# cr1m5onk1ng/text_similarity

Hardware: AMD Instinct MI355X
Metric: sentences/sec encoded + Mpairs/sec cosine top-k @ N=1M d=384 (higher is better)
Workload: dtype bf16 encoder / f16 selection / fp32 scores

## Files before the change

### include/tsim.h

```cpp
#ifndef TSIM_H
#define TSIM_H

#include <stddef.h>
#include <stdint.h>

#ifdef __cplusplus
extern "C" {
#endif

#define TSIM_OK 0
#define TSIM_EINVAL 1
#define TSIM_EHIP 2
#define TSIM_ENOMEM 3
#define TSIM_EUNSUPPORTED 4

#define TSIM_F32 0
#define TSIM_BF16 1

#define TSIM_ARCH_BERT 0
#define TSIM_ARCH_MPNET 1
#define TSIM_ARCH_ROBERTA 2

int tsim_version(void);
const char *tsim_last_error(void);
// ... 213 lines not shown
#define TSIM_POOL_MEAN_SQRT_LEN 3
#define TSIM_ACT_IDENTITY 0
#define TSIM_ACT_TANH 1
#define TSIM_ACT_RELU 2
typedef struct tsim_sentence_head {
    int32_t pool_mode;
    int32_t d_out;
    const float *dense_w, *dense_b;
    int32_t dense_act;
    int32_t normalize;
} tsim_sentence_head;

int tsim_encoder_forward_head(tsim_encoder *enc, const int32_t *tok_ids, const int32_t *tok_type, const int32_t *tok_pos,
                              const int32_t *tok_col, const int32_t *cu_seqlens, int32_t T, int32_t B, int32_t max_len,
                              const tsim_sentence_head *head, float *emb_f32, void *unit_f16, int ld_unit,
                              float *unit_rho_max, void *last_hidden_bf16, void *stream);

int tsim_encoder_forward_spans(tsim_encoder *enc, const int32_t *tok_ids, const int32_t *tok_type, const int32_t *tok_pos,
                               const int32_t *tok_col, const int32_t *cu_seqlens, int32_t T, int32_t B, int32_t max_len,
                               float *pooled_f32, void *unit_f16, int ld_unit, float *unit_rho_max,
                               void *last_hidden_bf16, float *logits_f32, const int32_t *span_seq, const int32_t *span_cu,
                               const int32_t *span_tok, int32_t S, int32_t n_span_tok, float *span_out_f32,
                               void *span_unit_f16, int ld_span_unit, float *span_rho_max, void *stream);

#define TSIM_ENC_ERR_TOKEN_ID 1
#define TSIM_ENC_ERR_POSITION 2
#define TSIM_ENC_ERR_MAX_LEN 4
#define TSIM_ENC_ERR_TOKEN_TYPE 8
#define TSIM_ENC_ERR_SPAN 16
int tsim_encoder_error_flags(tsim_encoder *enc, int32_t *flags_host, void *stream);

int tsim_chain_items_host(int blocks, int rem_blocks, int ntiles, int G, int b, int32_t *items, int cap);

int tsim_wordpiece_create(const char *vocab_text, const int64_t *vocab_offsets, int32_t vocab_size,
                          const char *continuing_prefix, int32_t unk_id, const int32_t *prefix_ids, int32_t n_prefix,
                          const int32_t *suffix_ids, int32_t n_suffix, int32_t lowercase, int32_t max_input_chars_per_word,
                          const char *added_text, const int64_t *added_offsets, int32_t n_added, void **handle);
void tsim_wordpiece_destroy(void *handle);
int tsim_wordpiece_encode(void *handle, const char *text, const int64_t *text_offsets, int64_t n, int32_t max_len,
                          int32_t n_threads, int32_t *out_ids, int64_t out_capacity, int32_t *out_lens, uint8_t *handled);

#ifdef __cplusplus
}
#endif
#endif
```

### text_similarity_amd/_lib.py

```python
from __future__ import annotations

import ctypes as C
import os

_HERE = os.path.dirname(os.path.abspath(__file__))
LIB_PATH = os.environ.get("TSIM_LIB") or os.path.join(_HERE, "libtsim.so")

TSIM_F32, TSIM_BF16 = 0, 1
TSIM_I32, TSIM_I64 = 2, 3
LIST_ST_ROW, LIST_ST_LIMS = 1, 2
IVF_ST_LIST, IVF_ST_OFF = 1, 2
IVF_SEG = 512
ARCH_BERT, ARCH_MPNET, ARCH_ROBERTA = 0, 1, 2
W_BF16, W_MXFP8 = 0, 1
POOL_MEAN, POOL_CLS, POOL_MAX, POOL_MEAN_SQRT_LEN = 0, 1, 2, 3
ACT_IDENTITY, ACT_TANH, ACT_RELU = 0, 1, 2
SPACE_COSINE, SPACE_DOT, SPACE_L2 = 0, 1, 2
ENC_ERR_SPAN = 16
RANGE_SLOT_CAP = 2048
RANGE_MERGE_MAX_LISTS = 64


class TsimError(RuntimeError):
    pass
# ... 108 lines not shown
                                    C.c_void_p, C.c_int64, C.c_void_p, C.c_size_t, C.c_void_p]),
    "tsim_int8_rescore_topk": (C.c_int, [C.c_void_p, C.c_int64, C.c_int64, C.c_void_p, C.c_int64, C.c_int64, C.c_int, C.c_void_p,
                                         C.c_int64, C.c_int, C.c_void_p, C.c_void_p, C.c_int64, C.c_void_p, C.c_void_p]),
    "tsim_ivf_scan_workspace_bytes": (C.c_size_t, [C.c_int64, C.c_int, C.c_int64, C.c_int]),
    "tsim_ivf_scan_topk": (C.c_int, [C.c_int, C.c_void_p, C.c_int64, C.c_int64, C.c_void_p, C.c_int64, C.c_int64, C.c_int, C.c_void_p,
                                     C.c_int64, C.c_void_p, C.c_void_p, C.c_int, C.c_int64, C.c_int, C.c_void_p, C.c_void_p, C.c_int64,
                                     C.c_void_p, C.c_void_p, C.c_size_t, C.c_void_p]),
    "tsim_cosine_topk": (C.c_int, [C.c_void_p, C.c_int64, C.c_void_p, C.c_int64, C.c_int, C.c_int, C.c_int,
                                   C.c_void_p, C.c_void_p, C.c_int64, C.c_void_p, C.c_size_t, C.c_void_p]),
    "tsim_time_next_topk": (None, [C.c_void_p, C.c_void_p]),
    "tsim_topk_merge": (C.c_int, [C.c_void_p, C.c_void_p, C.c_int, C.c_int64, C.c_int, C.c_int, C.c_void_p,
                                  C.c_void_p, C.c_void_p]),
    "tsim_topk_merge_strided": (C.c_int, [C.c_void_p, C.c_void_p, C.c_int, C.c_int64, C.c_int, C.c_int, C.c_int64, C.c_int64,
                                          C.c_void_p, C.c_void_p, C.c_void_p]),
    "tsim_wordpiece_create": (C.c_int, [C.c_char_p, C.c_void_p, C.c_int32, C.c_char_p, C.c_int32, C.c_void_p, C.c_int32, C.c_void_p,
                                        C.c_int32, C.c_int32, C.c_int32, C.c_char_p, C.c_void_p, C.c_int32, C.POINTER(C.c_void_p)]),
    "tsim_wordpiece_destroy": (None, [C.c_void_p]),
    "tsim_wordpiece_encode": (C.c_int, [C.c_void_p, C.c_char_p, C.c_void_p, C.c_int64, C.c_int32, C.c_int32, C.c_void_p, C.c_int64,
                                        C.c_void_p, C.c_void_p]),
    "tsim_cos_sim": (C.c_int, [C.c_void_p, C.c_int64, C.c_void_p, C.c_int64, C.c_int, C.c_void_p, C.c_void_p]),
    "tsim_mean_pool": (C.c_int, [C.c_void_p, C.c_int, C.c_void_p, C.c_int64, C.c_int, C.c_int, C.c_void_p,
                                 C.c_void_p]),
    "tsim_pool": (C.c_int, [C.c_void_p, C.c_int, C.c_void_p, C.c_int64, C.c_int, C.c_int, C.c_int, C.c_void_p, C.c_void_p]),
    "tsim_dense_rows": (C.c_int, [C.c_void_p, C.c_int64, C.c_int, C.c_void_p, C.c_void_p, C.c_int, C.c_int, C.c_int, C.c_void_p,
                                  C.c_void_p]),
    "tsim_quantize_mxfp8": (C.c_int, [C.c_void_p, C.c_int64, C.c_int, C.c_void_p, C.c_void_p, C.c_void_p]),
    "tsim_gemm_mxfp8": (C.c_int, [C.c_void_p, C.c_void_p, C.c_void_p, C.c_void_p, C.c_void_p, C.c_void_p, C.c_int, C.c_int,
                                  C.c_int, C.c_void_p]),
    "tsim_encoder_create": (C.c_int, [C.POINTER(EncoderConfigC), C.POINTER(EncoderWeightsC),
                                      C.POINTER(C.c_void_p)]),
    "tsim_encoder_destroy": (None, [C.c_void_p]),
    "tsim_encoder_error_flags": (C.c_int, [C.c_void_p, C.POINTER(C.c_int32), C.c_void_p]),
    "tsim_chain_items_host": (C.c_int, [C.c_int, C.c_int, C.c_int, C.c_int, C.c_int, C.POINTER(C.c_int32), C.c_int]),
    "tsim_encoder_forward": (C.c_int, [C.c_void_p, C.c_void_p, C.c_void_p, C.c_void_p, C.c_void_p, C.c_int32,
                                       C.c_int32, C.c_int32, C.c_void_p, C.c_void_p, C.c_int, C.c_void_p, C.c_void_p,
                                       C.c_void_p]),
    "tsim_encoder_set_token_types": (C.c_int, [C.c_void_p, C.c_void_p, C.c_int32]),
    "tsim_encoder_set_cls_head": (C.c_int, [C.c_void_p, C.c_void_p, C.c_void_p, C.c_void_p, C.c_void_p, C.c_int32]),
    "tsim_encoder_set_cls_head_act": (C.c_int, [C.c_void_p, C.c_void_p, C.c_void_p, C.c_void_p, C.c_void_p, C.c_int32, C.c_int32]),
    "tsim_encoder_forward_ex": (C.c_int, [C.c_void_p, C.c_void_p, C.c_void_p, C.c_void_p, C.c_void_p, C.c_void_p, C.c_int32,
                                          C.c_int32, C.c_int32, C.c_void_p, C.c_void_p, C.c_int, C.c_void_p, C.c_void_p,
                                          C.c_void_p, C.c_void_p]),
    "tsim_encoder_forward_head": (C.c_int, [C.c_void_p, C.c_void_p, C.c_void_p, C.c_void_p, C.c_void_p, C.c_void_p, C.c_int32,
                                            C.c_int32, C.c_int32, C.POINTER(SentenceHeadC), C.c_void_p, C.c_void_p, C.c_int,
                                            C.c_void_p, C.c_void_p, C.c_void_p]),
    "tsim_encoder_forward_spans": (C.c_int, [C.c_void_p, C.c_void_p, C.c_void_p, C.c_void_p, C.c_void_p, C.c_void_p, C.c_int32,
                                             C.c_int32, C.c_int32, C.c_void_p, C.c_void_p, C.c_int, C.c_void_p, C.c_void_p,
                                             C.c_void_p, C.c_void_p, C.c_void_p, C.c_void_p, C.c_int32, C.c_int32, C.c_void_p,
                                             C.c_void_p, C.c_int, C.c_void_p, C.c_void_p]),
}

DECLARED_SYMBOLS = tuple(_SIGS)


def lib() -> C.CDLL:
    global _lib
    if _lib is None:
        if not os.path.exists(LIB_PATH):
            raise TsimError(f"{LIB_PATH} not found: build it with `python -m text_similarity_amd.build` "
                            "(hipcc --offload-arch=gfx950); there is no CPU fallback")
        L = C.CDLL(LIB_PATH)
        for name, (res, args) in _SIGS.items():
            try:
                fn = getattr(L, name)
            except AttributeError:
                def fn(*a, _n=name, **kw):
# ... 15 lines not shown
```

### text_similarity_amd/csrc/encoder.hip

```cpp
#include <math.h>
#include <cmath>

#include <stdlib.h>
#include <string.h>

#include <vector>

#include <type_traits>
#include <utility>

#include "common.h"
#include "gemm_pp.h"

namespace tsim {

__device__ __forceinline__ int64_t packed_off(int64_t t, int f, int W) {
    return ((t >> 5) * (W >> 3) + (f >> 3)) * 256 + (t & 31) * 8 + (f & 7);
}
__device__ __forceinline__ int64_t group_off(int64_t t, int g, int W, int packed) {
    return packed ? packed_off(t, 8 * g, W) * 2 : (t * W + 8 * g) * 2;
}

template <int VPL, bool TYPED = false>
__global__ __launch_bounds__(256) void embed_ln_kernel(const int32_t *__restrict__ ids,
                                                       const int32_t *__restrict__ pos,
                                                       const float *__restrict__ word,
                                                       const float *__restrict__ pos_emb,
                                                       const float *__restrict__ type_tab,
                                                       const float *__restrict__ gamma,
                                                       const float *__restrict__ beta, float eps, int T, int H,
                                                       bf16_t *__restrict__ out, int vocab, int max_pos,
                                                       const int32_t *__restrict__ col, int max_len,
                                                       int *__restrict__ err_flags,
                                                       const int32_t *__restrict__ tok_type = nullptr, int n_types = 0) {
    const int lane = threadIdx.x & 63;
    const int t = blockIdx.x * 4 + (threadIdx.x >> 6);
    if (t >= T) return;
    int id = ids[t], ps = pos[t];
    int ty = 0;
    if constexpr (TYPED) ty = tok_type[t];
    int bad = 0;
    if (id < 0 || id >= vocab) { bad |= TSIM_ENC_ERR_TOKEN_ID; id = id < 0 ? 0 : vocab - 1; }
    if (ps < 0 || ps >= max_pos) { bad |= TSIM_ENC_ERR_POSITION; ps = ps < 0 ? 0 : max_pos - 1; }
    if (col[t] >= max_len || col[t] < 0) bad |= TSIM_ENC_ERR_MAX_LEN;
    if constexpr (TYPED) {
        if (ty < 0 || ty >= n_types) { bad |= TSIM_ENC_ERR_TOKEN_TYPE; ty = ty < 0 ? 0 : n_types - 1; }
    }
    if (bad && lane == 0) atomicOr(err_flags, bad);
    const float *w = word + (int64_t)id * H;
    const float *p = pos_emb + (int64_t)ps * H;
    const float *type_row = TYPED ? type_tab + (int64_t)ty * H : type_tab;
    float v[VPL], pv[VPL], tv[VPL];
#pragma unroll
    for (int i = 0; i < VPL; ++i) {
        v[i] = w[lane + i * 64];
        pv[i] = p[lane + i * 64];
    }
    if (type_row) {
#pragma unroll
        for (int i = 0; i < VPL; ++i) tv[i] = type_row[lane + i * 64];
    }
    float s = 0.f;
#pragma unroll
    for (int i = 0; i < VPL; ++i) {
        float a = v[i];
        if (type_row) a += tv[i];
        a += pv[i];
        v[i] = a;
        s += a;
// ... 1057 lines not shown
            }
            ++st;
            ring = ring + 1 == X2_NSTAGE ? 0 : ring + 1;
            if (st >= 3) carry = 0;
        }
        old_m0 = m0;
        old_n0 = n0;
        old_rowoff = (uint32_t)(m0 >> 5) * (uint32_t)(N2 * 64) + 16u * r2 + 512u * h2;
    };
    int item = 0;
    run_item(accA, accB, item++, std::false_type{});
    for (; item + 2 <= part.n; item += 2) {
        run_item(accB, accA, item, std::true_type{});
        run_item(accA, accB, item + 1, std::true_type{});
    }
    const bool lastA = item >= part.n;
    if (!lastA) run_item(accB, accA, item, std::true_type{});
    wait_vmcnt<0>();
    auto flush = [&](f32x16 (&a)[X2_NSUB]) __attribute__((always_inline)) {
#pragma unroll
        for (int g = 0; g < X2_NSUB; ++g) {
            uint32_t pk[8];
#pragma unroll
            for (int ks = 0; ks < 8; ++ks) pk[ks] = finish2(a[g][2 * ks], a[g][2 * ks + 1]);
            store_half(pk, old_m0, old_n0 + g * 32, std::integral_constant<int, 0>{});
            store_half(pk, old_m0, old_n0 + g * 32, std::integral_constant<int, 2>{});
        }
    };
    if (lastA) flush(accA); else flush(accB);
}

template <int DH, bool REL, bool PK = false>
__global__ __launch_bounds__(256) __attribute__((amdgpu_waves_per_eu(DH <= 32 ? 6 : 4))) void attention_kernel(const bf16_t *__restrict__ qkv,
                                                        const int32_t *__restrict__ cu, const int32_t *__restrict__ col,
                                                        const float *__restrict__ relb, int relw, int H,
                                                        int heads, float scale, bf16_t *__restrict__ ctx, int B, int xcd_map) {
    constexpr int KS = DH / 16;
    constexpr int OT = (DH + 31) / 32;
    constexpr int ROWB = DH * 2 < 64 ? 64 : DH * 2;
    __shared__ __attribute__((aligned(16))) char vimg[4 * 32 * ROWB];
    typedef __attribute__((ext_vector_type(4))) short s16x4;
    const int lane = threadIdx.x & 63;
    const int wave = __builtin_amdgcn_readfirstlane(threadIdx.x >> 6);
    int seq = blockIdx.x;
    if (xcd_map) {
        seq = (blockIdx.x & 7) * (gridDim.x >> 3) + (blockIdx.x >> 3);
        if (seq >= B) return;
    }
    const int head = blockIdx.y * 4 + wave, qb = blockIdx.z;
    const int t0 = cu[seq], S = cu[seq + 1] - t0;
    if (qb * 32 >= S || head >= heads) return;
    const int r = lane & 31, h = lane >> 5;
    const int64_t H3 = 3 * (int64_t)H;
    const int qi = qb * 32 + r;
    const int tq = t0 + (qi < S ? qi : S - 1);

    bf16x8 qf[KS];
    {
        const bf16_t *qp = PK ? qkv + packed_off(tq, head * DH + 8 * h, (int)H3) : qkv + tq * H3 + head * DH + 8 * h;
#pragma unroll
        for (int s = 0; s < KS; ++s) {
            qf[s] = *reinterpret_cast<const bf16x8 *>(qp + (PK ? 2 * 256 : 16) * s);
        }
    }
    const int qcol = REL ? col[tq] : 0;
    f32x16 o[OT];
#pragma unroll
    for (int ob = 0; ob < OT; ++ob)
#pragma unroll
        for (int g = 0; g < 16; ++g) o[ob][g] = 0.f;
    float m = -INFINITY, l = 0.f;

    for (int k0 = 0; k0 < S; k0 += 32) {
        const int kr = k0 + r;
        const int tk = t0 + (kr < S ? kr : S - 1);
        f32x16 sc;
#pragma unroll
        for (int g = 0; g < 16; ++g) sc[g] = 0.f;
        constexpr int CH = DH / 16;
        uint4 vr[CH];
        {
            const bf16_t *kp = PK ? qkv + packed_off(tk, H + head * DH + 8 * h, (int)H3) : qkv + tk * H3 + H + head * DH + 8 * h;
            const bf16_t *vsrc = PK ? qkv + packed_off(tk, 2 * H + head * DH + h * (DH / 2), (int)H3)
                                    : qkv + tk * H3 + 2 * H + head * DH + h * (DH / 2);
// ... 491 lines not shown
    }
};

}

using namespace tsim;

struct tsim_encoder {
    tsim_encoder_config cfg;
    int Tp = 0;
    float *word = nullptr, *pos = nullptr, *type0 = nullptr, *emb_g = nullptr, *emb_b = nullptr, *relb = nullptr;
    int relw = 0;
    int n_types = 0;
    float *head_wpT = nullptr, *head_bp = nullptr, *head_wc = nullptr, *head_bc = nullptr;
    int n_labels = 0;
    int head_act = TSIM_ACT_TANH;
    struct Layer {
        bf16_t *wqkv, *wo, *w1, *w2;
        bf16_t *pqkv = nullptr, *po = nullptr;
        bf16_t *lo = nullptr, *l2 = nullptr;
        bf16_t *lo32 = nullptr, *l232 = nullptr;
        uint8_t *qqkv = nullptr, *qo = nullptr, *q1 = nullptr, *q2 = nullptr;
        uint8_t *sqkv = nullptr, *so = nullptr, *s1 = nullptr, *s2 = nullptr;
        float *bqkv, *bo, *b1, *b2, *g1, *be1, *g2, *be2;
    };
    std::vector<Layer> layers;
    std::vector<void *> allocs;
    bf16_t *x0 = nullptr, *x1 = nullptr, *qkv = nullptr, *ctx = nullptr, *h1 = nullptr;
    float *ybuf = nullptr;
    float *lnimg = nullptr;
    float *head_x = nullptr;
    uint8_t *aq = nullptr, *as = nullptr, *hq = nullptr, *hs = nullptr;
    int *err_flags = nullptr;
};

namespace tsim {

static int dev_alloc(tsim_encoder *e, size_t bytes, void **out) {
    void *p = nullptr;
    hipError_t err = hipMalloc(&p, bytes);
    if (err != hipSuccess) return fail(TSIM_ENOMEM, "hipMalloc(%zu) failed: %s", bytes, hipGetErrorString(err));
    e->allocs.push_back(p);
    *out = p;
    return TSIM_OK;
}

static int upload_f32(tsim_encoder *e, const float *h, size_t n, float **out) {
    int rc = dev_alloc(e, n * 4, (void **)out);
    if (rc) return rc;
    TSIM_HIP_CHECK(hipMemcpy(*out, h, n * 4, hipMemcpyHostToDevice));
    return TSIM_OK;
}

static int upload_bf16(tsim_encoder *e, const std::vector<const float *> &parts, size_t n_each, bf16_t **out) {
    std::vector<uint16_t> tmp(n_each * parts.size());
    for (size_t p = 0; p < parts.size(); ++p)
        for (size_t i = 0; i < n_each; ++i) tmp[p * n_each + i] = host_f32_to_bf16(parts[p][i]);
    int rc = dev_alloc(e, tmp.size() * 2, (void **)out);
    if (rc) return rc;
    TSIM_HIP_CHECK(hipMemcpy(*out, tmp.data(), tmp.size() * 2, hipMemcpyHostToDevice));
    return TSIM_OK;
}

static uint8_t host_f32_to_e4m3(float v) {
    const uint8_t sign = std::signbit(v) ? 0x80 : 0;
    const double a = std::fabs((double)v);
// ... 400 lines not shown
                    after_rows = true;
                }
                if (M <= LS_MAX_BLOCKS * 32 && K % (16 * LT_PF) == 0)
                    return ln_tail_gemm(X, Wimg32, bias, res, gamma, beta, eps, out, M, K, st, xpacked, lnimg, respacked, opacked);
            }
            const int mt = (M + 127) / 128, full = (mt / 256) * 256, rem = mt - full;
            auto main_launch = [&](int rows) {
                return launch_gemm<128, 384, 64, 2, 4, EPI_RES_LN>(X, W, bias, res, gamma, beta, eps, out, rows, N, K, st, Wimg, xpacked, respacked, opacked);
            };
            if (rem > 0 && rem <= 96 && (full > 0 || after_rows)) {
                const int m_main = full * 128;
                if (full > 0) {
                    int rc = main_launch(m_main);
                    if (rc) return rc;
                }
                return launch_gemm<64, 384, 64, 2, 4, EPI_RES_LN>(X + (int64_t)m_main * K, W, bias, res + (int64_t)m_main * N,
                                                                  gamma, beta, eps, out + (int64_t)m_main * N, M - m_main, N, K, st, Wimg, xpacked, respacked, opacked);
            }
            return main_launch(M);
        }
        case 768: return launch_gemm<64, 768, 32, 1, 8, EPI_RES_LN>(X, W, bias, res, gamma, beta, eps, out, M, N, K, st);
        case 64: return launch_gemm<128, 64, 64, 4, 2, EPI_RES_LN>(X, W, bias, res, gamma, beta, eps, out, M, N, K, st);
        default: return fail(TSIM_EUNSUPPORTED, "encoder: hidden size %d has no fused LayerNorm GEMM (64, 384, 768)", N);
    }
}

}

extern "C" int tsim_chain_items_host(int blocks, int rem_blocks, int ntiles, int G, int b, int32_t *items, int cap) {
    if (blocks != G || rem_blocks < 0 || ntiles <= 0 || G <= 0 || b < 0 || b >= G || (cap > 0 && !items)) return -1;
    const ChainPart p = chain_part(G, rem_blocks, ntiles, b);
    for (int i = 0; i < p.n && i < cap; ++i) items[i] = chain_item(p, G, ntiles, b, i);
    return p.n;
}

extern "C" int tsim_encoder_create(const tsim_encoder_config *cfg, const tsim_encoder_weights_host *w,
                                   tsim_encoder **out) {
    TSIM_REQUIRE(cfg && w && out, "encoder_create: null pointer");
    const int H = cfg->hidden, F = cfg->ffn, L = cfg->num_layers;
    TSIM_REQUIRE(H == 64 || H == 384 || H == 768 || H == 1024, "encoder_create: hidden=%d unsupported (64, 384, 768, 1024)", H);
    TSIM_REQUIRE(cfg->heads > 0 && H % cfg->heads == 0, "encoder_create: heads=%d does not divide hidden=%d", cfg->heads, H);
    const int dh = H / cfg->heads;
    TSIM_REQUIRE(dh == 16 || dh == 32 || dh == 64, "encoder_create: head_dim=%d unsupported (16, 32, 64)", dh);
    TSIM_REQUIRE(F > 0 && F % 64 == 0 && L > 0 && cfg->max_tokens > 0 && cfg->max_seqs > 0, "encoder_create: bad ffn/layers/capacity");
    if (H != 64 && F < 128)
        return fail(TSIM_EUNSUPPORTED, "encoder_create: ffn=%d unsupported at hidden=%d (a multiple of 64, at least 128)", F, H);
    TSIM_REQUIRE(cfg->arch == TSIM_ARCH_BERT || cfg->arch == TSIM_ARCH_MPNET || cfg->arch == TSIM_ARCH_ROBERTA, "encoder_create: unknown arch");
    TSIM_REQUIRE(w->word_emb && w->pos_emb && w->emb_ln_g && w->emb_ln_b && w->layers, "encoder_create: missing weights");
    TSIM_REQUIRE(cfg->arch != TSIM_ARCH_MPNET || w->rel_bias, "encoder_create: MPNet needs rel_bias");
    const bool mx = cfg->weight_dtype == TSIM_W_MXFP8;
    TSIM_REQUIRE(cfg->weight_dtype == TSIM_W_BF16 || mx, "encoder_create: unknown weight_dtype %d", cfg->weight_dtype);
    if (mx && !(gemm_pp_mx_supported(H, H) && gemm_pp_mx_supported(3 * H, H) && gemm_pp_mx_supported(F, H) && gemm_pp_mx_supported(H, F)))
        return fail(TSIM_EUNSUPPORTED, "encoder_create: MXFP8 projections need hidden and ffn to be multiples of 256 (got %d, %d)", H, F);
    tsim_encoder *e = new tsim_encoder();
    e->cfg = *cfg;
    e->Tp = (cfg->max_tokens + 127) / 128 * 128 + 128;
    int rc = TSIM_OK;
    auto bail = [&](int code) {
        tsim_encoder_destroy(e);
        return code;
    };
    if ((rc = upload_f32(e, w->word_emb, (size_t)cfg->vocab * H, &e->word))) return bail(rc);
    if ((rc = upload_f32(e, w->pos_emb, (size_t)cfg->max_pos * H, &e->pos))) return bail(rc);
    if (w->type_emb && (rc = upload_f32(e, w->type_emb, H, &e->type0))) return bail(rc);
    if ((rc = upload_f32(e, w->emb_ln_g, H, &e->emb_g))) return bail(rc);
    if ((rc = upload_f32(e, w->emb_ln_b, H, &e->emb_b))) return bail(rc);
// ... 61 lines not shown
        if ((rc = upload_f32(e, lw.ln1_g, H, &d.g1))) return bail(rc);
        if ((rc = upload_f32(e, lw.ln1_b, H, &d.be1))) return bail(rc);
        if ((rc = upload_f32(e, lw.ln2_g, H, &d.g2))) return bail(rc);
        if ((rc = upload_f32(e, lw.ln2_b, H, &d.be2))) return bail(rc);
    }
    const size_t Tp = e->Tp;
    struct { bf16_t **p; size_t n; } acts[] = {{&e->x0, Tp * H}, {&e->x1, Tp * H}, {&e->qkv, Tp * 3 * H},
                                               {&e->ctx, Tp * H}, {&e->h1, Tp * F}};
    for (auto &a : acts) {
        if ((rc = dev_alloc(e, a.n * 2, (void **)a.p))) return bail(rc);
        if (hipMemset(*a.p, 0, a.n * 2) != hipSuccess) return bail(fail(TSIM_EHIP, "hipMemset failed"));
    }
    if (H >= 512 && H % 256 == 0 && gemm_pp_supported(H, H)) {
        if ((rc = dev_alloc(e, Tp * H * 4, (void **)&e->ybuf))) return bail(rc);
        if (hipMemset(e->ybuf, 0, Tp * H * 4) != hipSuccess) return bail(fail(TSIM_EHIP, "hipMemset failed"));
    }
    if (!mx && H == 384 && F % 64 == 0) {
        const size_t blocks = (Tp + 31) / 32 < (size_t)LS_MAX_BLOCKS ? (Tp + 31) / 32 : (size_t)LS_MAX_BLOCKS;
        const size_t bytes = blocks * 4 * 12 * 64 * 16;
        if ((rc = dev_alloc(e, bytes, (void **)&e->lnimg))) return bail(rc);
        if (hipMemset(e->lnimg, 0, bytes) != hipSuccess) return bail(fail(TSIM_EHIP, "hipMemset failed"));
    }
    if ((size_t)cfg->max_seqs * H * 4 > Tp * 3 * H * 2 && (rc = dev_alloc(e, (size_t)cfg->max_seqs * H * 4, (void **)&e->head_x)))
        return bail(rc);
    if (mx) {
        struct { uint8_t **p; size_t n; } qb[] = {{&e->aq, Tp * H}, {&e->as, Tp * H / 32}, {&e->hq, Tp * F}, {&e->hs, Tp * F / 32}};
        for (auto &a : qb) {
            if ((rc = dev_alloc(e, a.n, (void **)a.p))) return bail(rc);
            if (hipMemset(*a.p, 0, a.n) != hipSuccess) return bail(fail(TSIM_EHIP, "hipMemset failed"));
        }
    }
    if ((rc = dev_alloc(e, 256, (void **)&e->err_flags))) return bail(rc);
    if (hipMemset(e->err_flags, 0, 256) != hipSuccess) return bail(fail(TSIM_EHIP, "hipMemset failed"));
    if (hipDeviceSynchronize() != hipSuccess) return bail(fail(TSIM_EHIP, "sync after upload failed"));
    *out = e;
    return TSIM_OK;
}

extern "C" int tsim_encoder_error_flags(tsim_encoder *e, int32_t *flags_host, void *stream) {
    TSIM_REQUIRE(e && flags_host, "encoder_error_flags: null pointer");
    hipStream_t st = reinterpret_cast<hipStream_t>(stream);
    TSIM_HIP_CHECK(hipMemcpyAsync(flags_host, e->err_flags, 4, hipMemcpyDeviceToHost, st));
    TSIM_HIP_CHECK(hipMemsetAsync(e->err_flags, 0, 4, st));
    TSIM_HIP_CHECK(hipStreamSynchronize(st));
    return TSIM_OK;
}

extern "C" int tsim_quantize_mxfp8(const void *x_bf16, int64_t rows, int K, void *q_out, void *scale_out, void *stream) {
    TSIM_REQUIRE(x_bf16 && q_out && scale_out, "quantize_mxfp8: null pointer");
    TSIM_REQUIRE(rows >= 0 && K > 0, "quantize_mxfp8: bad shape rows=%lld K=%d", (long long)rows, K);
    return quant_mx(static_cast<const bf16_t *>(x_bf16), rows, K, static_cast<uint8_t *>(q_out),
                    static_cast<uint8_t *>(scale_out), reinterpret_cast<hipStream_t>(stream));
}

extern "C" int tsim_gemm_mxfp8(const void *xq, const void *xs, const void *wq, const void *ws, const float *bias,
                               float *out_f32, int M, int N, int K, void *stream) {
    TSIM_REQUIRE(xq && xs && wq && ws && bias && out_f32, "gemm_mxfp8: null pointer");
    TSIM_REQUIRE(M >= 0 && N > 0 && K > 0, "gemm_mxfp8: bad shape M=%d N=%d K=%d", M, N, K);
    return gemm_pp_mx(PP_EPI_F32, static_cast<const uint8_t *>(xq), static_cast<const uint8_t *>(xs),
                      static_cast<const uint8_t *>(wq), 0, static_cast<const uint8_t *>(ws), bias, out_f32, nullptr, M, N, K,
                      reinterpret_cast<hipStream_t>(stream));
}

#ifdef TSIM_PP_STAMPS
extern "C" int tsim_debug_xr_stamps(unsigned long long *out16, int reset) {
    if (hipMemcpyFromSymbol(out16, HIP_SYMBOL(tsim::g_xr_stamps), 128) != hipSuccess) return 1;
// ... 48 lines not shown

extern "C" int tsim_encoder_forward(tsim_encoder *e, const int32_t *tok_ids, const int32_t *tok_pos,
                                    const int32_t *tok_col, const int32_t *cu_seqlens, int32_t T, int32_t B,
                                    int32_t max_len, float *pooled_f32, void *unit_bf16, int ld_unit, float *unit_rho_max,
                                    void *last_hidden_bf16, void *stream) {
    return tsim_encoder_forward_ex(e, tok_ids, nullptr, tok_pos, tok_col, cu_seqlens, T, B, max_len, pooled_f32, unit_bf16, ld_unit,
                                   unit_rho_max, last_hidden_bf16, nullptr, stream);
}

extern "C" int tsim_encoder_forward_ex(tsim_encoder *e, const int32_t *tok_ids, const int32_t *tok_type, const int32_t *tok_pos,
                                       const int32_t *tok_col, const int32_t *cu_seqlens, int32_t T, int32_t B,
                                       int32_t max_len, float *pooled_f32, void *unit_bf16, int ld_unit, float *unit_rho_max,
                                       void *last_hidden_bf16, float *logits_f32, void *stream) {
    TSIM_REQUIRE(e && cu_seqlens && (T == 0 || (tok_ids && tok_pos)), "encoder_forward: null pointer");
    TSIM_REQUIRE(!tok_type || e->n_types > 0, "encoder_forward: tok_type given but no token-type table was set "
                 "(tsim_encoder_set_token_types)");
    TSIM_REQUIRE(!logits_f32 || e->n_labels > 0, "encoder_forward: logits requested but no classification head was set "
                 "(tsim_encoder_set_cls_head)");
    TSIM_REQUIRE(T >= 0 && B >= 0 && T <= e->cfg.max_tokens && B <= e->cfg.max_seqs,
                 "encoder_forward: T=%d B=%d exceed capacity (%d tokens, %d sequences)", T, B, e->cfg.max_tokens, e->cfg.max_seqs);
    const int pos_span = max_len + (e->cfg.arch != TSIM_ARCH_BERT ? e->cfg.pad_id + 1 : 0);
    TSIM_REQUIRE(max_len >= 0 && pos_span <= e->cfg.max_pos,
                 "encoder_forward: sequences of %d tokens need position rows up to %d, the table has %d", max_len, pos_span - 1,
                 e->cfg.max_pos);
    TSIM_REQUIRE(!unit_bf16 || ld_unit >= e->cfg.hidden, "encoder_forward: ld_unit < hidden");
    TSIM_REQUIRE(!unit_bf16 || e->cfg.hidden <= 768, "encoder_forward: unit rows need a width <= 768 (got %d)", e->cfg.hidden);
    if (B == 0) return TSIM_OK;
    hipStream_t st = reinterpret_cast<hipStream_t>(stream);
    const tsim_encoder_config &c = e->cfg;
    const int H = c.hidden, F = c.ffn, dh = H / c.heads;
    const bool mx = c.weight_dtype == TSIM_W_MXFP8;
    int rc;
    if (T > 0) {
        const unsigned g = (unsigned)((T + 3) / 4);
        const int32_t *colp = tok_col ? tok_col : tok_pos;
        const int col_limit = tok_col || c.arch == TSIM_ARCH_BERT ? max_len : c.max_pos;
#define EMBED(V) hipLaunchKernelGGL(embed_ln_kernel<V>, dim3(g), dim3(256), 0, st, tok_ids, tok_pos, e->word, e->pos, e->type0, e->emb_g, e->emb_b, c.ln_eps, T, H, e->x0, c.vocab, c.max_pos, colp, col_limit, e->err_flags, nullptr, 0)
#define EMBED_T(V) hipLaunchKernelGGL((embed_ln_kernel<V, true>), dim3(g), dim3(256), 0, st, tok_ids, tok_pos, e->word, e->pos, e->type0, e->emb_g, e->emb_b, c.ln_eps, T, H, e->x0, c.vocab, c.max_pos, colp, col_limit, e->err_flags, tok_type, e->n_types)
        if (tok_type) {
            if (H == 64) EMBED_T(1); else if (H == 384) EMBED_T(6); else if (H == 768) EMBED_T(12); else EMBED_T(16);
        } else if (H == 64) EMBED(1); else if (H == 384) EMBED(6); else if (H == 768) EMBED(12); else EMBED(16);
#undef EMBED_T
#undef EMBED
        TSIM_HIP_CHECK(hipGetLastError());
        const float scale = 1.0f / sqrtf((float)dh);
        const bool rel = c.arch == TSIM_ARCH_MPNET;
        const bool pk = !mx && !rel && use_packed_layout(H, F);
        const int32_t *col = rel ? (tok_col ? tok_col : tok_pos) : nullptr;
        const int qblocks = (max_len + 31) / 32 > 0 ? (max_len + 31) / 32 : 1;
        const dim3 agrid((unsigned)(((B + 7) / 8) * 8), (unsigned)((c.heads + 3) / 4), (unsigned)qblocks);
        bool qkv_chained = false;
        for (int l = 0; l < c.num_layers; ++l) {
            const tsim_encoder::Layer &L = e->layers[l];
            const bool x0pk = pk && l > 0, x0pk_next = pk && l + 1 < c.num_layers;
            if (mx) {
                if (l == 0 && (rc = quant_mx(e->x0, T, H, e->aq, e->as, st))) return rc;
                if ((rc = gemm_pp_mx(PP_EPI_BIAS, e->aq, e->as, L.qqkv, 1, L.sqkv, L.bqkv, e->qkv, nullptr, T, 3 * H, H, st))) return rc;
            } else if (pk) {
                if (!qkv_chained) {
                    rc = x0pk ? gemm_xres2<EPI_BIAS, true, true>(e->x0, L.wqkv, L.bqkv, e->qkv, T, 3 * H, st)
                              : gemm_xres2<EPI_BIAS, true>(e->x0, L.wqkv, L.bqkv, e->qkv, T, 3 * H, st);
                    if (rc) return rc;
                }
            } else if ((rc = gemm_plain<EPI_BIAS>(e->x0, L.wqkv, L.pqkv, L.bqkv, e->qkv, T, 3 * H, H, st))) return rc;
#define ATT(D)                                                                                                 \
    do {                                                                                                       \
        if (rel)                                                                                               \
            hipLaunchKernelGGL((attention_kernel<D, true>), agrid, dim3(256), 0, st, e->qkv, cu_seqlens, col,  \
                               e->relb, e->relw, H, c.heads, scale, e->ctx, B, 1);                                         \
        else if (pk)                                                                                           \
            hipLaunchKernelGGL((attention_kernel<D, false, true>), agrid, dim3(256), 0, st, e->qkv, cu_seqlens, col, \
                               e->relb, e->relw, H, c.heads, scale, e->ctx, B, 1);                                         \
        else                                                                                                   \
            hipLaunchKernelGGL((attention_kernel<D, false>), agrid, dim3(256), 0, st, e->qkv, cu_seqlens, col, \
                               e->relb, e->relw, H, c.heads, scale, e->ctx, B, 1);                                         \
    } while (0)
            if (dh == 16) ATT(16); else if (dh == 32) ATT(32); else ATT(64);
#undef ATT
            TSIM_HIP_CHECK(hipGetLastError());
            if (mx) {
                if ((rc = quant_mx(e->ctx, T, H, e->aq, e->as, st))) return rc;
                if ((rc = gemm_pp_mx(PP_EPI_F32, e->aq, e->as, L.qo, 1, L.so, L.bo, e->ybuf, nullptr, T, H, H, st))) return rc;
                if ((rc = res_ln_rows(e->ybuf, e->x0, L.g1, L.be1, c.ln_eps, e->x1, e->aq, e->as, T, H, st))) return rc;
                if ((rc = gemm_pp_mx(PP_EPI_GELU_MX, e->aq, e->as, L.q1, 1, L.s1, L.b1, e->hq, e->hs, T, F, H, st))) return rc;
                if ((rc = gemm_pp_mx(PP_EPI_F32, e->hq, e->hs, L.q2, 1, L.s2, L.b2, e->ybuf, nullptr, T, H, F, st))) return rc;
                if ((rc = res_ln_rows(e->ybuf, e->x1, L.g2, L.be2, c.ln_eps, e->x0, e->aq, e->as, T, H, st))) return rc;
                continue;
            }
            const int chain_blocks = pk && F <= 1536 && ln_rows_blocks(T) % 256 == 0 ? ln_rows_blocks(T) : 0;
            if (chain_blocks > 0 && L.lo32) {
                if ((rc = gemm_res_ln(e->ctx, L.wo, L.po, L.bo, e->x0, L.g1, L.be1, c.ln_eps, e->x1, T, H, H, e->ybuf, st, L.lo, L.lo32, false, e->lnimg, x0pk, pk, true))) return rc;
                if ((rc = ln_rows_xres2<EPI_GELU>(e->ctx, L.lo32, L.bo, e->x0, L.g1, L.be1, c.ln_eps, e->x1, chain_blocks, H, false, x0pk,
                                                  L.w1, L.b1, e->h1, T, F, st))) return rc;
            } else {
                if ((rc = gemm_res_ln(e->ctx, L.wo, L.po, L.bo, e->x0, L.g1, L.be1, c.ln_eps, e->x1, T, H, H, e->ybuf, st, L.lo, L.lo32, false, e->lnimg, x0pk, pk))) return rc;
                if (pk) {
                    if ((rc = gemm_xres2<EPI_GELU, true, true>(e->x1, L.w1, L.b1, e->h1, T, F, st))) return rc;
                } else if ((rc = gemm_plain<EPI_GELU>(e->x1, L.w1, nullptr, L.b1, e->h1, T, F, H, st))) return rc;
            }
            qkv_chained = chain_blocks > 0 && L.l232 && x0pk_next;
            if (qkv_chained) {
                const tsim_encoder::Layer &Ln = e->layers[l + 1];
                if ((rc = gemm_res_ln(e->h1, L.w2, nullptr, L.b2, e->x1, L.g2, L.be2, c.ln_eps, e->x0, T, H, F, e->ybuf, st, L.l2, L.l232, pk, e->lnimg, pk, true, true))) return rc;
                if ((rc = ln_rows_xres2<EPI_BIAS>(e->h1, L.l232, L.b2, e->x1, L.g2, L.be2, c.ln_eps, e->x0, chain_blocks, F, true, true,
                                                  Ln.wqkv, Ln.bqkv, e->qkv, T, 3 * H, st))) return rc;
            } else if ((rc = gemm_res_ln(e->h1, L.w2, nullptr, L.b2, e->x1, L.g2, L.be2, c.ln_eps, e->x0, T, H, F, e->ybuf, st, L.l2, L.l232, pk, e->lnimg, pk, x0pk_next))) return rc;
        }
        if (last_hidden_bf16)
// ... 90 lines not shown
```

Baseline: 910,300.

## Compact attention grid into a device-built list of live query blocks

The first workgroup of the embedding kernel now builds, with a prefix scan over cu_seqlens, a compact list of (seq, query-block, t0, S) records. The records are interleaved across the 8 XCDs. The attention kernel then launches one workgroup per live record instead of a padded B x heads x max_qblocks grid, where most blocks exited early on short sequences. This removes idle workgroup launches and the per-block cu lookups. In exchange, block 0 of the embed kernel does serial scan work, and an extra device buffer plus a host helper are added.

Result: no change. 917,200 (median of 6 runs) (+0.8%).

```diff
diff --git a/include/tsim.h b/include/tsim.h
--- a/include/tsim.h
+++ b/include/tsim.h
@@ -269,6 +269,8 @@
 
 int tsim_chain_items_host(int blocks, int rem_blocks, int ntiles, int G, int b, int32_t *items, int cap);
 
+int tsim_attn_blocks_host(const int32_t *cu, int B, int32_t *out, int cap);
+
 int tsim_wordpiece_create(const char *vocab_text, const int64_t *vocab_offsets, int32_t vocab_size,
                           const char *continuing_prefix, int32_t unk_id, const int32_t *prefix_ids, int32_t n_prefix,
                           const int32_t *suffix_ids, int32_t n_suffix, int32_t lowercase, int32_t max_input_chars_per_word,
diff --git a/text_similarity_amd/_lib.py b/text_similarity_amd/_lib.py
--- a/text_similarity_amd/_lib.py
+++ b/text_similarity_amd/_lib.py
@@ -164,6 +164,7 @@
     "tsim_encoder_destroy": (None, [C.c_void_p]),
     "tsim_encoder_error_flags": (C.c_int, [C.c_void_p, C.POINTER(C.c_int32), C.c_void_p]),
     "tsim_chain_items_host": (C.c_int, [C.c_int, C.c_int, C.c_int, C.c_int, C.c_int, C.POINTER(C.c_int32), C.c_int]),
+    "tsim_attn_blocks_host": (C.c_int, [C.POINTER(C.c_int32), C.c_int, C.POINTER(C.c_int32), C.c_int]),
     "tsim_encoder_forward": (C.c_int, [C.c_void_p, C.c_void_p, C.c_void_p, C.c_void_p, C.c_void_p, C.c_int32,
                                        C.c_int32, C.c_int32, C.c_void_p, C.c_void_p, C.c_int, C.c_void_p, C.c_void_p,
                                        C.c_void_p]),
diff --git a/text_similarity_amd/csrc/encoder.hip b/text_similarity_amd/csrc/encoder.hip
--- a/text_similarity_amd/csrc/encoder.hip
+++ b/text_similarity_amd/csrc/encoder.hip
@@ -19,6 +19,64 @@
 }
 __device__ __forceinline__ int64_t group_off(int64_t t, int g, int W, int packed) {
     return packed ? packed_off(t, 8 * g, W) * 2 : (t * W + 8 * g) * 2;
+}
+
+struct AttnBlock { int32_t seq, qb, t0, S; };
+static_assert(sizeof(AttnBlock) == 16, "one 16-byte load per workgroup");
+__host__ __device__ inline int attn_blocks_of(int S, int qcap) {
+    const int nb = S > 0 ? (S + 31) / 32 : 0;
+    return nb < qcap ? nb : qcap;
+}
+__host__ __device__ inline int attn_blocks_count(const int32_t *cu, int s0, int s1, int qcap) {
+    int c = 0;
+    for (int s = s0; s < s1; ++s) c += attn_blocks_of(cu[s + 1] - cu[s], qcap);
+    return c;
+}
+__host__ __device__ inline int attn_block_slot(int n, int e) {
+    const int c8 = (n + 7) / 8;
+    return (e % c8) * 8 + e / c8;
+}
+__host__ __device__ inline bool attn_slot_dead(int n, int i) {
+    const int c8 = (n + 7) / 8;
+    return i / 8 >= c8 || (i % 8) * c8 + i / 8 >= n;
+}
+__host__ __device__ inline void attn_blocks_fill(const int32_t *cu, int s0, int s1, int qcap, int e0, int n, AttnBlock *out) {
+    int e = e0;
+    for (int s = s0; s < s1 && e < n; ++s) {
+        const int t0 = cu[s], S = cu[s + 1] - t0, nb = attn_blocks_of(S, qcap);
+        for (int qb = 0; qb < nb && e < n; ++qb, ++e) out[attn_block_slot(n, e)] = AttnBlock{s, qb, t0, S};
+    }
+}
+inline int attn_grid_slots(int64_t T, int64_t B, int64_t max_len) {
+    const int64_t qcap = max_len > 0 ? (max_len + 31) / 32 : 1, by_len = B * qcap, by_tok = (T + 31 * B) / 32;
+    const int64_t U = by_len < by_tok ? by_len : by_tok;
+    return (int)((U + 7) / 8 * 8);
+}
+__device__ __forceinline__ void attn_blocks_build(const int32_t *__restrict__ cu, int B, int qcap, AttnBlock *__restrict__ out, int cap) {
+    __shared__ int wsum[4];
+    const int tid = threadIdx.x, lane = tid & 63, wave = tid >> 6;
+    const int per = (B + 255) / 256;
+    const int s0 = tid * per < B ? tid * per : B, s1 = s0 + per < B ? s0 + per : B;
+    const int cnt = attn_blocks_count(cu, s0, s1, qcap);
+    int inc = cnt;
+#pragma unroll
+    for (int d = 1; d < 64; d <<= 1) {
+        const int v = __shfl_up(inc, d, 64);
+        if (lane >= d) inc += v;
+    }
+    if (lane == 63) wsum[wave] = inc;
+    __syncthreads();
+    int base = 0, total = 0;
+#pragma unroll
+    for (int w = 0; w < 4; ++w) {
+        const int v = wsum[w];
+        base += w < wave ? v : 0;
+        total += v;
+    }
+    const int n = total < cap ? total : cap;
+    attn_blocks_fill(cu, s0, s1, qcap, base + inc - cnt, n, out);
+    for (int i = tid; i < cap; i += 256)
+        if (attn_slot_dead(n, i)) out[i] = AttnBlock{-1, 0, 0, 0};
 }
 
 template <int VPL, bool TYPED = false>
@@ -32,9 +90,15 @@
                                                        bf16_t *__restrict__ out, int vocab, int max_pos,
                                                        const int32_t *__restrict__ col, int max_len,
                                                        int *__restrict__ err_flags,
-                                                       const int32_t *__restrict__ tok_type = nullptr, int n_types = 0) {
+                                                       const int32_t *__restrict__ tok_type, int n_types,
+                                                       const int32_t *__restrict__ cu, int B, int qcap,
+                                                       AttnBlock *__restrict__ blocks, int block_slots) {
+    if (blockIdx.x == 0) {
+        attn_blocks_build(cu, B, qcap, blocks, block_slots);
+        return;
+    }
     const int lane = threadIdx.x & 63;
-    const int t = blockIdx.x * 4 + (threadIdx.x >> 6);
+    const int t = (blockIdx.x - 1) * 4 + (threadIdx.x >> 6);
     if (t >= T) return;
     int id = ids[t], ps = pos[t];
     int ty = 0;
@@ -1158,9 +1222,9 @@
 
 template <int DH, bool REL, bool PK = false>
 __global__ __launch_bounds__(256) __attribute__((amdgpu_waves_per_eu(DH <= 32 ? 6 : 4))) void attention_kernel(const bf16_t *__restrict__ qkv,
-                                                        const int32_t *__restrict__ cu, const int32_t *__restrict__ col,
+                                                        const int4 *__restrict__ blocks, const int32_t *__restrict__ col,
                                                         const float *__restrict__ relb, int relw, int H,
-                                                        int heads, float scale, bf16_t *__restrict__ ctx, int B, int xcd_map) {
+                                                        int heads, float scale, bf16_t *__restrict__ ctx) {
     constexpr int KS = DH / 16;
     constexpr int OT = (DH + 31) / 32;
     constexpr int ROWB = DH * 2 < 64 ? 64 : DH * 2;
@@ -1168,14 +1232,11 @@
     typedef __attribute__((ext_vector_type(4))) short s16x4;
     const int lane = threadIdx.x & 63;
     const int wave = __builtin_amdgcn_readfirstlane(threadIdx.x >> 6);
-    int seq = blockIdx.x;
-    if (xcd_map) {
-        seq = (blockIdx.x & 7) * (gridDim.x >> 3) + (blockIdx.x >> 3);
-        if (seq >= B) return;
-    }
-    const int head = blockIdx.y * 4 + wave, qb = blockIdx.z;
-    const int t0 = cu[seq], S = cu[seq + 1] - t0;
-    if (qb * 32 >= S || head >= heads) return;
+    const int4 blk = blocks[blockIdx.x];
+    if (blk.x < 0) return;
+    const int head = blockIdx.y * 4 + wave, qb = blk.y;
+    const int t0 = blk.z, S = blk.w;
+    if (head >= heads) return;
     const int r = lane & 31, h = lane >> 5;
     const int64_t H3 = 3 * (int64_t)H;
     const int qi = qb * 32 + r;
@@ -1733,6 +1794,8 @@
     float *head_x = nullptr;
     uint8_t *aq = nullptr, *as = nullptr, *hq = nullptr, *hs = nullptr;
     int *err_flags = nullptr;
+    tsim::AttnBlock *attn_blocks = nullptr;
+    int attn_slots = 0;
 };
 
 namespace tsim {
@@ -2199,6 +2262,21 @@
     const ChainPart p = chain_part(G, rem_blocks, ntiles, b);
     for (int i = 0; i < p.n && i < cap; ++i) items[i] = chain_item(p, G, ntiles, b, i);
     return p.n;
+}
+
+extern "C" int tsim_attn_blocks_host(const int32_t *cu, int B, int32_t *out, int cap) {
+    if (!cu || B < 0 || cap < 0 || cap % 8 != 0 || (cap > 0 && !out)) return -1;
+    for (int s = 0; s < B; ++s)
+        if (cu[s + 1] < cu[s]) return -1;
+    const int qcap = INT32_MAX;
+    const long long total = [&] { long long c = 0; for (int s = 0; s < B; ++s) c += attn_blocks_of(cu[s + 1] - cu[s], qcap); return c; }();
+    if (total > INT32_MAX) return -1;
+    const int n = (int)total < cap ? (int)total : cap;
+    AttnBlock *rec = reinterpret_cast<AttnBlock *>(out);
+    attn_blocks_fill(cu, 0, B, qcap, 0, n, rec);
+    for (int i = 0; i < cap; ++i)
+        if (attn_slot_dead(n, i)) rec[i] = AttnBlock{-1, 0, 0, 0};
+    return (int)total;
 }
 
 extern "C" int tsim_encoder_create(const tsim_encoder_config *cfg, const tsim_encoder_weights_host *w,
@@ -2326,6 +2404,9 @@
     }
     if ((rc = dev_alloc(e, 256, (void **)&e->err_flags))) return bail(rc);
     if (hipMemset(e->err_flags, 0, 256) != hipSuccess) return bail(fail(TSIM_EHIP, "hipMemset failed"));
+    e->attn_slots = attn_grid_slots(cfg->max_tokens, cfg->max_seqs, cfg->max_pos);
+    if ((rc = dev_alloc(e, (size_t)e->attn_slots * sizeof(AttnBlock), (void **)&e->attn_blocks))) return bail(rc);
+    if (hipMemset(e->attn_blocks, 0xff, (size_t)e->attn_slots * sizeof(AttnBlock)) != hipSuccess) return bail(fail(TSIM_EHIP, "hipMemset failed"));
     if (hipDeviceSynchronize() != hipSuccess) return bail(fail(TSIM_EHIP, "sync after upload failed"));
     *out = e;
     return TSIM_OK;
@@ -2440,11 +2521,14 @@
     const bool mx = c.weight_dtype == TSIM_W_MXFP8;
     int rc;
     if (T > 0) {
-        const unsigned g = (unsigned)((T + 3) / 4);
+        const int qblocks = (max_len + 31) / 32 > 0 ? (max_len + 31) / 32 : 1;
+        const int aslots = attn_grid_slots(T, B, max_len);
+        TSIM_REQUIRE(aslots <= e->attn_slots, "encoder_forward: block list of %d slots, %d allocated", aslots, e->attn_slots);
+        const unsigned g = (unsigned)((T + 3) / 4) + 1;
         const int32_t *colp = tok_col ? tok_col : tok_pos;
         const int col_limit = tok_col || c.arch == TSIM_ARCH_BERT ? max_len : c.max_pos;
-#define EMBED(V) hipLaunchKernelGGL(embed_ln_kernel<V>, dim3(g), dim3(256), 0, st, tok_ids, tok_pos, e->word, e->pos, e->type0, e->emb_g, e->emb_b, c.ln_eps, T, H, e->x0, c.vocab, c.max_pos, colp, col_limit, e->err_flags, nullptr, 0)
-#define EMBED_T(V) hipLaunchKernelGGL((embed_ln_kernel<V, true>), dim3(g), dim3(256), 0, st, tok_ids, tok_pos, e->word, e->pos, e->type0, e->emb_g, e->emb_b, c.ln_eps, T, H, e->x0, c.vocab, c.max_pos, colp, col_limit, e->err_flags, tok_type, e->n_types)
+#define EMBED(V) hipLaunchKernelGGL(embed_ln_kernel<V>, dim3(g), dim3(256), 0, st, tok_ids, tok_pos, e->word, e->pos, e->type0, e->emb_g, e->emb_b, c.ln_eps, T, H, e->x0, c.vocab, c.max_pos, colp, col_limit, e->err_flags, nullptr, 0, cu_seqlens, B, qblocks, e->attn_blocks, aslots)
+#define EMBED_T(V) hipLaunchKernelGGL((embed_ln_kernel<V, true>), dim3(g), dim3(256), 0, st, tok_ids, tok_pos, e->word, e->pos, e->type0, e->emb_g, e->emb_b, c.ln_eps, T, H, e->x0, c.vocab, c.max_pos, colp, col_limit, e->err_flags, tok_type, e->n_types, cu_seqlens, B, qblocks, e->attn_blocks, aslots)
         if (tok_type) {
             if (H == 64) EMBED_T(1); else if (H == 384) EMBED_T(6); else if (H == 768) EMBED_T(12); else EMBED_T(16);
         } else if (H == 64) EMBED(1); else if (H == 384) EMBED(6); else if (H == 768) EMBED(12); else EMBED(16);
@@ -2455,8 +2539,8 @@
         const bool rel = c.arch == TSIM_ARCH_MPNET;
         const bool pk = !mx && !rel && use_packed_layout(H, F);
         const int32_t *col = rel ? (tok_col ? tok_col : tok_pos) : nullptr;
-        const int qblocks = (max_len + 31) / 32 > 0 ? (max_len + 31) / 32 : 1;
-        const dim3 agrid((unsigned)(((B + 7) / 8) * 8), (unsigned)((c.heads + 3) / 4), (unsigned)qblocks);
+        const int4 *ablocks = reinterpret_cast<const int4 *>(e->attn_blocks);
+        const dim3 agrid((unsigned)aslots, (unsigned)((c.heads + 3) / 4));
         bool qkv_chained = false;
         for (int l = 0; l < c.num_layers; ++l) {
             const tsim_encoder::Layer &L = e->layers[l];
@@ -2474,14 +2558,14 @@
 #define ATT(D)                                                                                                 \
     do {                                                                                                       \
         if (rel)                                                                                               \
-            hipLaunchKernelGGL((attention_kernel<D, true>), agrid, dim3(256), 0, st, e->qkv, cu_seqlens, col,  \
-                               e->relb, e->relw, H, c.heads, scale, e->ctx, B, 1);                                         \
+            hipLaunchKernelGGL((attention_kernel<D, true>), agrid, dim3(256), 0, st, e->qkv, ablocks, col,     \
+                               e->relb, e->relw, H, c.heads, scale, e->ctx);                                   \
         else if (pk)                                                                                           \
-            hipLaunchKernelGGL((attention_kernel<D, false, true>), agrid, dim3(256), 0, st, e->qkv, cu_seqlens, col, \
-                               e->relb, e->relw, H, c.heads, scale, e->ctx, B, 1);                                         \
+            hipLaunchKernelGGL((attention_kernel<D, false, true>), agrid, dim3(256), 0, st, e->qkv, ablocks, col, \
+                               e->relb, e->relw, H, c.heads, scale, e->ctx);                                   \
         else                                                                                                   \
-            hipLaunchKernelGGL((attention_kernel<D, false>), agrid, dim3(256), 0, st, e->qkv, cu_seqlens, col, \
-                               e->relb, e->relw, H, c.heads, scale, e->ctx, B, 1);                                         \
+            hipLaunchKernelGGL((attention_kernel<D, false>), agrid, dim3(256), 0, st, e->qkv, ablocks, col,    \
+                               e->relb, e->relw, H, c.heads, scale, e->ctx);                                   \
     } while (0)
             if (dh == 16) ATT(16); else if (dh == 32) ATT(32); else ATT(64);
 #undef ATT
```
